# lucidrains/ring-attention-pytorch

Measured on AMD Instinct MI355X. Metric: attn_tflops, higher is better.
Workload: dtype bf16; 1 GPU; model=ring_flash_attn (non-causal, d_head 64), global_batch=1, seq_len=8192, seq_per_gpu=8192, heads=8, kv_heads=8, d_head=64, parallelism=ring1, hipgraph=True

## Files before the change

### ring_attention_amd/csrc/attn_bwd.hip

```cpp

#include <hip/hip_runtime.h>
#include <hip/hip_bf16.h>
#include <cstdint>

#include "attn_common.h"

namespace ring_attn {

template <int D>
struct DqLds {
    static constexpr int KVB = kvblk(D);
    __align__(16) __bf16 k[2][KVB * D];
    __align__(16) __bf16 v[2][KVB * D];
    unsigned char kmask[2][KVB];
};

template <int D, bool SOFTCLAMP, bool PAIRED, bool BIAS = false>
__global__ __launch_bounds__(512, 2)
void attn_bwd_dq_kernel(BwdParams p) {
    constexpr int DBLK = D / 32;
    constexpr int KSTEPS = D / 16;
    constexpr int DQ_KVBLK = kvblk(D);
    constexpr int DQ_NBLK = DQ_KVBLK / 32;

    __shared__ DqLds<D> lds;

    const int tid = threadIdx.x;
    const int lane = tid & 63;
    const int wid = tid >> 6;
    const int l31 = lane & 31;
    const int lhi = lane >> 5;

    const int bh = blockIdx.y;
    const int b = bh / p.h;
    const int h = bh % p.h;
    const int hk = h % p.hk;

    const int n_pit = PAIRED
        ? (p.paired - 1 - (int)blockIdx.x == (int)blockIdx.x ? 1 : 2) : 1;
    for (int pit = 0; pit < n_pit; ++pit) {
    const int qtile = PAIRED
        ? (pit == 0 ? (int)blockIdx.x : p.paired - 1 - (int)blockIdx.x)
        : (p.desc ? p.desc[(long)blockIdx.x * 3] : (int)blockIdx.x);
    if (PAIRED && pit == 1) {
        __syncthreads();
    }

    auto dq_body = [&]() {
    const BwdParams P = p;
    const long i = (long)qtile * ROWS_WG + wid * 32 + l31;
    const bool row_valid = i < P.nq;
    const long ic = row_valid ? i : 0;

    const __bf16* qbase = (const __bf16*)P.q + ((long)b * P.nq + ic) * P.h * D + (long)h * D;
    const __bf16* dobase = (const __bf16*)P.dout + ((long)b * P.nq + ic) * P.h * D + (long)h * D;
    bf16x8 qf[KSTEPS], dof[KSTEPS];
    #pragma unroll
    for (int ks = 0; ks < KSTEPS; ++ks) {
        qf[ks] = *(const bf16x8*)(qbase + ks * 16 + lhi * 8);
        dof[ks] = *(const bf16x8*)(dobase + ks * 16 + lhi * 8);
    }
    const float lse_i = P.lse[((long)b * P.h + h) * P.nq + ic] * LOG2E;
    const float delta_i = P.delta[((long)b * P.h + h) * P.nq + ic];

    f32x16 dq_acc[DBLK];
    #pragma unroll
    for (int db = 0; db < DBLK; ++db) dq_acc[db] = f32x16{};

    const Mask M = mask_of(P);
    const long wg_i_min = (long)qtile * ROWS_WG;
    const long wg_i_max = min((long)(qtile + 1) * ROWS_WG, P.nq) - 1;
    const long wg_q_min = M.qpos(wg_i_min);
    const long wg_q_max = M.qpos(wg_i_max);
    const long qpos_i = M.qpos(i);
    TileRange tr = M.kv_tile_range(wg_i_min, wg_i_max, P.nk, DQ_KVBLK);
    if (P.split > 1) tr = split_share(tr, P.split, (int)blockIdx.z);
    if (!PAIRED && P.desc)
        tr = {P.desc[(long)blockIdx.x * 3 + 1], P.desc[(long)blockIdx.x * 3 + 2]};
    const int t_lo = tr.lo, t_hi = tr.hi;

    constexpr int CH = D * 2 / 16;
    constexpr int KCHUNKS = DQ_KVBLK * CH;
    constexpr int KREGS = (KCHUNKS + 511) / 512;
    const __bf16* kbase = (const __bf16*)P.k + ((long)b * P.nk) * P.hk * D + (long)hk * D;
    const __bf16* vbase = (const __bf16*)P.v + ((long)b * P.nk) * P.hk * D + (long)hk * D;
    const unsigned char* mbase = P.kmask ? (const unsigned char*)P.kmask + (long)b * P.nk : nullptr;

    const long kv_row_stride = (long)P.hk * D;
    const long tile_stride = DQ_KVBLK * kv_row_stride;
    const __bf16* kptr = kbase + (long)t_lo * tile_stride
        + (tid / CH) * kv_row_stride + (tid % CH) * 8;
    const __bf16* vptr = vbase + (long)t_lo * tile_stride
        + (tid / CH) * kv_row_stride + (tid % CH) * 8;
    long j0_next = (long)t_lo * DQ_KVBLK;

    uint4 kst[KREGS], vst[KREGS];
    unsigned char mst = 1;

    auto load_tile = [&]() {
        const long j0 = j0_next;
        const long jmax = min(j0 + DQ_KVBLK, P.nk) - 1;
        const bool full = jmax - j0 == DQ_KVBLK - 1;
        #pragma unroll
        for (int r = 0; r < KREGS; ++r) {
            int c = tid + r * 512;
            if (c < KCHUNKS) {
                long off = (long)(r * (512 / CH)) * kv_row_stride;
                bool okr = full || (j0 + c / CH) <= jmax;
                kst[r] = okr ? *(const uint4*)(kptr + off) : uint4{0, 0, 0, 0};
                vst[r] = okr ? *(const uint4*)(vptr + off) : uint4{0, 0, 0, 0};
            }
        }
        if (mbase && tid < DQ_KVBLK)
            mst = (j0 + tid <= jmax) ? mbase[j0 + tid] : 0;
        kptr += tile_stride; vptr += tile_stride;
        j0_next += DQ_KVBLK;
    };

    auto write_tile = [&](int par) {
        #pragma unroll
        for (int r = 0; r < KREGS; ++r) {
            int c = tid + r * 512;
            if (c < KCHUNKS) {
                int row = c / CH, ch = c % CH;
                *(uint4*)(lds.k[par] + row * D + swz<D / 8>(row, ch) * 8) = kst[r];
                *(uint4*)(lds.v[par] + row * D + swz<D / 8>(row, ch) * 8) = vst[r];
            }
        }
        if (mbase && tid < DQ_KVBLK) lds.kmask[par][tid] = mst;
    };

    const float scale2 = P.scale * LOG2E;
    if (t_lo < t_hi) {
        load_tile();
        write_tile(t_lo & 1);
        if (t_lo + 1 < t_hi) load_tile();
    }

    for (int t = t_lo; t < t_hi; ++t) {
        const int par = t & 1;
        const long j0 = (long)t * DQ_KVBLK;
        const long jmax = min(j0 + DQ_KVBLK, P.nk) - 1;
        const bool full_tile = !BIAS &&
            (jmax - j0 == DQ_KVBLK - 1) &&
            M.uncut(wg_q_min, wg_q_max, j0, jmax) &&
            !P.kmask;

        __syncthreads();

        alignas(16) uint32_t pk[DQ_NBLK * 8];
        __builtin_amdgcn_s_setprio(1);
        #pragma unroll
        for (int kb = 0; kb < DQ_NBLK; ++kb) {
            f32x16 s = f32x16{}, dp = f32x16{};
            int krow = kb * 32 + l31;
            #pragma unroll
            for (int ks = 0; ks < KSTEPS; ++ks) {
                int chunk = ks * 2 + lhi;
                bf16x8 kfr = *(const bf16x8*)(lds.k[par] + krow * D + swz<D / 8>(krow, chunk) * 8);
                bf16x8 vfr = *(const bf16x8*)(lds.v[par] + krow * D + swz<D / 8>(krow, chunk) * 8);
                s = __builtin_amdgcn_mfma_f32_32x32x16_bf16(kfr, qf[ks], s, 0, 0, 0);
                dp = __builtin_amdgcn_mfma_f32_32x32x16_bf16(vfr, dof[ks], dp, 0, 0, 0);
            }
            if (full_tile && row_valid) {
                #pragma unroll
                for (int x2 = 0; x2 < 8; ++x2) {
                    float dse[2];
                    #pragma unroll
                    for (int e = 0; e < 2; ++e) {
                        int r = 2 * x2 + e;
                        float x, dtanh = 1.f;
                        if constexpr (SOFTCLAMP) {
                            float inv_v = __builtin_amdgcn_rcpf(P.softclamp_value);
                            float th = fast_tanhf(s[r] * P.scale * inv_v);
                            x = P.softclamp_value * th * LOG2E;
                            dtanh = 1.f - th * th;
                        } else {
                            x = __builtin_fmaf(s[r], scale2, -lse_i);
                        }
                        float pv = __builtin_amdgcn_exp2f(SOFTCLAMP ? x - lse_i : x);
                        dse[e] = pv * (dp[r] - delta_i);
                        if constexpr (SOFTCLAMP) dse[e] *= dtanh;
                    }
                    pk[kb * 8 + x2] = pack_bf16x2(dse[0], dse[1]);
                }
            } else {
                #pragma unroll
                for (int x2 = 0; x2 < 8; ++x2) {
                    float dse[2];
                    #pragma unroll
                    for (int e = 0; e < 2; ++e) {
                        int r = 2 * x2 + e;
                        long jj = j0 + kb * 32 + (r & 3) + 8 * (r >> 2) + 4 * lhi;
                        float x, dtanh = 1.f;
                        if constexpr (SOFTCLAMP) {
                            float inv_v = __builtin_amdgcn_rcpf(P.softclamp_value);
                            float th = fast_tanhf(s[r] * P.scale * inv_v);
                            x = P.softclamp_value * th * LOG2E;
                            dtanh = 1.f - th * th;
                        } else {
                            x = s[r] * scale2;
                        }
                        bool ok = row_valid && jj <= jmax;
                        if constexpr (BIAS) {
                            if (ok) {
                                const long bi = P.bias_mat
                                    ? (((long)b * P.h + h) * P.nq + ic) * P.nk + jj
                                    : ((long)b * P.h + h) * P.nk + jj;
                                x += P.bias[bi] * LOG2E;
                            }
                        }
                        ok = M.attends(qpos_i, jj, ok);
                        if (P.kmask) ok = ok && lds.kmask[par][jj - j0];
                        float pv = ok ? __builtin_amdgcn_exp2f(
                            SOFTCLAMP ? x - lse_i : x - lse_i) : 0.f;
                        dse[e] = pv * (dp[r] - delta_i);
                        if constexpr (SOFTCLAMP) dse[e] *= dtanh;
                    }
                    pk[kb * 8 + x2] = pack_bf16x2(dse[0], dse[1]);
                }
            }
        }
        __builtin_amdgcn_s_setprio(0);

        if (t + 1 < t_hi) write_tile(par ^ 1);
        if (t + 2 < t_hi) load_tile();

        {
            const int f15 = lane & 15;
            const int g16 = (lane >> 4) & 1;
            const unsigned kb_lds = (unsigned)(uintptr_t)
                (__attribute__((address_space(3))) __bf16*)lds.k[par];
            __builtin_amdgcn_s_setprio(1);
            unsigned long long ktr[DBLK][DQ_NBLK * 2][2];
            #pragma unroll
            for (int db = 0; db < DBLK; ++db) {
                const int dg = db * 32 + g16 * 16 + 4 * (f15 & 3);
                #pragma unroll
                for (int ks = 0; ks < DQ_NBLK * 2; ++ks) {
                    #pragma unroll
                    for (int half = 0; half < 2; ++half) {
                        const int kv = ks * 16 + 4 * lhi + 8 * half + (f15 >> 2);
                        const int c = (dg / 8) ^ (kv & (CH < 8 ? CH - 1 : 7));
                        const unsigned a = kb_lds
                            + (unsigned)(kv * (D * 2) + c * 16 + (dg % 8) * 2);
                        asm volatile("ds_read_b64_tr_b16 %0, %1"
                                     : "=&v"(ktr[db][ks][half]) : "v"(a) : "memory");
                    }
                }
            }
            asm volatile("s_waitcnt lgkmcnt(0)" ::: "memory");
            __builtin_amdgcn_sched_barrier(0);
            #pragma unroll
            for (int db = 0; db < DBLK; ++db)
                #pragma unroll
                for (int ks = 0; ks < DQ_NBLK * 2; ++ks) {
                    bf16x8 ktf;
                    *(unsigned long long*)&ktf = ktr[db][ks][0];
                    *((unsigned long long*)&ktf + 1) = ktr[db][ks][1];
                    dq_acc[db] = __builtin_amdgcn_mfma_f32_32x32x16_bf16(
                        ktf, *(const bf16x8*)(pk + 4 * ks), dq_acc[db], 0, 0, 0);
                }
            __builtin_amdgcn_s_setprio(0);
        }
    }

    if (!row_valid) return;
    #pragma unroll
    for (int db = 0; db < DBLK; ++db) dq_acc[db] *= P.scale;
    if (P.dq_bf) {
        __bf16* dqb = (__bf16*)P.dq_bf + ((long)b * P.nq + i) * P.h * D + (long)h * D;
        #pragma unroll
        for (int db = 0; db < DBLK; ++db)
            #pragma unroll
            for (int g = 0; g < 4; ++g) {
                f32x4 v4 = {dq_acc[db][4 * g], dq_acc[db][4 * g + 1],
                            dq_acc[db][4 * g + 2], dq_acc[db][4 * g + 3]};
                *(bf16x4*)(dqb + db * 32 + 8 * g + 4 * lhi) =
                    __builtin_convertvector(v4, bf16x4);
            }
        return;
    }
    float* dqp = P.dq + ((long)b * P.nq + i) * P.h * D + (long)h * D;
    #pragma unroll
    for (int db = 0; db < DBLK; ++db)
        #pragma unroll
        for (int r = 0; r < 16; ++r) {
            int d = db * 32 + (r & 3) + 8 * (r >> 2) + 4 * lhi;
            if (P.split > 1 || P.desc) atomicAdd(dqp + d, dq_acc[db][r]);
            else if (P.accumulate) dqp[d] += dq_acc[db][r];
            else dqp[d] = dq_acc[db][r];
        }
    };
    dq_body();
    }
}

static constexpr int KVROWS_WAVE = 32;
static_assert(ROWS_WG == 8 * KVROWS_WAVE);

template <int D, int QT>
struct DkvLds {
    __align__(16) __bf16 q[2][QT * D];
    __align__(16) __bf16 qt[2][D * QT];
    __align__(16) __bf16 do_[2][QT * D];
    __align__(16) __bf16 dot[2][D * QT];
    __align__(16) float lse[2][QT];
    __align__(16) float delta[2][QT];
};


template <int D, int QT, bool SOFTCLAMP, bool PAIRED, bool BIAS = false>
__global__ __launch_bounds__(512, 2)
void attn_bwd_dkv_kernel(BwdParams p) {
    static_assert(D % 32 == 0 && QT % 32 == 0);
    constexpr int DBLK = D / 32;
    constexpr int KSTEPS = D / 16;
    constexpr int QBLKS = QT / 32;
    constexpr int TM = (QT / 8 - 1) < 7 ? (QT / 8 - 1) : 7;

    __shared__ DkvLds<D, QT> lds;

    const int tid = threadIdx.x;
    const int lane = tid & 63;
    const int wid = tid >> 6;
    const int l31 = lane & 31;
    const int lhi = lane >> 5;

    const int bhk = blockIdx.y;
    const int b = bhk / p.hk;
    const int hkh = bhk % p.hk;

    const int n_pit = PAIRED
        ? (p.paired - 1 - (int)blockIdx.x == (int)blockIdx.x ? 1 : 2) : 1;
    for (int pit = 0; pit < n_pit; ++pit) {
    const int kvtile = PAIRED
        ? (pit == 0 ? (int)blockIdx.x : p.paired - 1 - (int)blockIdx.x)
        : (p.desc ? p.desc[(long)blockIdx.x * 3] : (int)blockIdx.x);
    if (PAIRED && pit == 1) {
        __syncthreads();
    }

    auto dkv_body = [&]() {
    const BwdParams P = p;
    const long j0_wg = (long)kvtile * ROWS_WG;
    const long jmax = min(j0_wg + ROWS_WG, P.nk) - 1;
    const long j = j0_wg + wid * KVROWS_WAVE + l31;
    const bool col_valid = j <= jmax;
    const long jc = col_valid ? j : j0_wg;

    const __bf16* kb = (const __bf16*)P.k + ((long)b * P.nk + jc) * P.hk * D + (long)hkh * D;
    const __bf16* vb = (const __bf16*)P.v + ((long)b * P.nk + jc) * P.hk * D + (long)hkh * D;
    bf16x8 kf[KSTEPS], vf[KSTEPS];
    #pragma unroll
    for (int ks = 0; ks < KSTEPS; ++ks) {
        kf[ks] = *(const bf16x8*)(kb + ks * 16 + lhi * 8);
        vf[ks] = *(const bf16x8*)(vb + ks * 16 + lhi * 8);
    }
    unsigned char kmask_own = 1;
    if (P.kmask) kmask_own = col_valid ? ((const unsigned char*)P.kmask)[(long)b * P.nk + j] : 0;

    f32x16 dv_acc[DBLK], dk_acc[DBLK];
    #pragma unroll
    for (int db = 0; db < DBLK; ++db) { dv_acc[db] = f32x16{}; dk_acc[db] = f32x16{}; }
    const float scale2 = P.scale * LOG2E;

    const Mask M = mask_of(P);

    for (int g = 0; g < P.group; ++g) {
        if (g > 0) __syncthreads();
        const int h = hkh + g * P.hk;
        const float* lse_row = P.lse + ((long)b * P.h + h) * P.nq;
        const float* delta_row = P.delta + ((long)b * P.h + h) * P.nq;
        const __bf16* qg = (const __bf16*)P.q + ((long)b * P.nq) * P.h * D + (long)h * D;
        const __bf16* dog = (const __bf16*)P.dout + ((long)b * P.nq) * P.h * D + (long)h * D;

        TileRange tr = M.q_tile_range(j0_wg, jmax, P.nq, QT);
        if (P.split > 1) tr = split_share(tr, P.split, (int)blockIdx.z);
        if (!PAIRED && P.desc)
            tr = {P.desc[(long)blockIdx.x * 3 + 1], P.desc[(long)blockIdx.x * 3 + 2]};
        const int t0 = tr.lo, t1 = tr.hi;

        constexpr int CH = D * 2 / 16;
        constexpr int QCHUNKS = QT * CH;
        constexpr int QREGS = (QCHUNKS + 511) / 512;
        constexpr int TPAIRS = (QT / 2) * (D / 8);
        constexpr int TREGS = (TPAIRS + 511) / 512;
        uint4 qst[QREGS], dost[QREGS];
        bf16x8 qtv_a[TREGS], qtv_b[TREGS], dov_a[TREGS], dov_b[TREGS];
        float lse_st = 0.f, delta_st = 0.f;
        long t_next = t0;

        auto load_qtile = [&]() {
            const long i0 = t_next * QT;
            const long imax_ = min(i0 + QT, P.nq) - 1;
            const bool full = imax_ - i0 == QT - 1;
            #pragma unroll
            for (int r = 0; r < QREGS; ++r) {
                int c = tid + r * 512;
                if (c < QCHUNKS) {
                    long gr = i0 + c / CH;
                    int ch = c % CH;
                    const __bf16* src = qg + gr * P.h * D + ch * 8;
                    const __bf16* srd = dog + gr * P.h * D + ch * 8;
                    bool okr = full || gr <= imax_;
                    qst[r] = okr ? *(const uint4*)src : uint4{0, 0, 0, 0};
                    dost[r] = okr ? *(const uint4*)srd : uint4{0, 0, 0, 0};
                }
            }
            #pragma unroll
            for (int r = 0; r < TREGS; ++r) {
                int c = tid + r * 512;
                if (c < TPAIRS) {
                    int jp = c % (QT / 2);
                    int d0 = (c / (QT / 2)) * 8;
                    long ra = i0 + jp * 2;
                    bool oka = full || ra <= imax_;
                    bool okb = full || ra + 1 <= imax_;
                    const __bf16* qa_ = qg + ra * P.h * D + d0;
                    const __bf16* da_ = dog + ra * P.h * D + d0;
                    qtv_a[r] = oka ? *(const bf16x8*)qa_ : bf16x8{};
                    qtv_b[r] = okb ? *(const bf16x8*)(qa_ + P.h * D) : bf16x8{};
                    dov_a[r] = oka ? *(const bf16x8*)da_ : bf16x8{};
                    dov_b[r] = okb ? *(const bf16x8*)(da_ + P.h * D) : bf16x8{};
                }
            }
            if (tid < QT) {
                long gi = i0 + tid;
                bool okl = gi <= imax_;
                lse_st = okl ? lse_row[gi] * LOG2E : 0.f;
                delta_st = okl ? delta_row[gi] : 0.f;
            }
            ++t_next;
        };

        auto write_qtile = [&](int par) {
            #pragma unroll
            for (int r = 0; r < QREGS; ++r) {
                int c = tid + r * 512;
                if (c < QCHUNKS) {
                    int row = c / CH, ch = c % CH;
                    *(uint4*)(lds.q[par] + row * D + swz<D / 8>(row, ch) * 8) = qst[r];
                    *(uint4*)(lds.do_[par] + row * D + swz<D / 8>(row, ch) * 8) = dost[r];
                }
            }
            #pragma unroll
            for (int r = 0; r < TREGS; ++r) {
                int c = tid + r * 512;
                if (c < TPAIRS) {
                    int jp = kperm_pair(c % (QT / 2));
                    int d0 = (c / (QT / 2)) * 8;
                    #pragma unroll
                    for (int e = 0; e < 8; ++e) {
                        int dd = d0 + e;
                        int byte_off = dd * QT * 2 + ((jp * 4) ^ ((dd & TM) << 4));
                        __bf16 pq[2] = {qtv_a[r][e], qtv_b[r][e]};
                        __bf16 pd[2] = {dov_a[r][e], dov_b[r][e]};
                        *(uint32_t*)((char*)lds.qt[par] + byte_off) = *(uint32_t*)pq;
                        *(uint32_t*)((char*)lds.dot[par] + byte_off) = *(uint32_t*)pd;
                    }
                }
            }
            if (tid < QT) {
                lds.lse[par][tid] = lse_st;
                lds.delta[par][tid] = delta_st;
            }
        };

        if (t0 < t1) {
            load_qtile();
            write_qtile(t0 & 1);
            if (t0 + 1 < t1) load_qtile();
        }

        for (int t = t0; t < t1; ++t) {
            const int par = t & 1;
            const long i0 = (long)t * QT;
            const long imax = min(i0 + QT, P.nq) - 1;
            const bool full_tile = !BIAS &&
                (imax - i0 == QT - 1) &&
                M.uncut(M.qpos(i0), M.qpos(imax), j0_wg, jmax) &&
                !P.kmask;

            __syncthreads();

            if (t + 1 < t1) write_qtile(par ^ 1);
            if (t + 2 < t1) load_qtile();

            #pragma unroll
            for (int qb = 0; qb < QBLKS; ++qb) {
                f32x16 s2 = f32x16{}, dp = f32x16{};
                #pragma unroll
                for (int ks = 0; ks < KSTEPS; ++ks) {
                    int qrow = qb * 32 + l31;
                    int chunk = ks * 2 + lhi;
                    bf16x8 qa = *(const bf16x8*)(lds.q[par] + qrow * D + swz<D / 8>(qrow, chunk) * 8);
                    bf16x8 da = *(const bf16x8*)(lds.do_[par] + qrow * D + swz<D / 8>(qrow, chunk) * 8);
                    s2 = __builtin_amdgcn_mfma_f32_32x32x16_bf16(qa, kf[ks], s2, 0, 0, 0);
                    dp = __builtin_amdgcn_mfma_f32_32x32x16_bf16(da, vf[ks], dp, 0, 0, 0);
                }

                alignas(16) uint32_t p_pk[8], ds_pk[8];
                if (full_tile && col_valid) {
                    #pragma unroll
                    for (int x2 = 0; x2 < 8; ++x2) {
                        float pe[2], dse[2];
                        f32x4 lse4, delta4;
                        {
                            int base = qb * 32 + 8 * (x2 >> 1) + 4 * lhi;
                            lse4 = *(const f32x4*)(lds.lse[par] + base);
                            delta4 = *(const f32x4*)(lds.delta[par] + base);
                        }
                        #pragma unroll
                        for (int e = 0; e < 2; ++e) {
                            int r = 2 * x2 + e;
                            float x, dtanh = 1.f;
                            if constexpr (SOFTCLAMP) {
                                float inv_v = __builtin_amdgcn_rcpf(P.softclamp_value);
                                float th = fast_tanhf(s2[r] * P.scale * inv_v);
                                x = P.softclamp_value * th * LOG2E;
                                dtanh = 1.f - th * th;
                            } else {
                                x = __builtin_fmaf(s2[r], scale2, -lse4[r & 3]);
                            }
                            float pv = __builtin_amdgcn_exp2f(SOFTCLAMP ? x - lse4[r & 3] : x);
                            pe[e] = pv;
                            dse[e] = pv * (dp[r] - delta4[r & 3]);
                            if constexpr (SOFTCLAMP) dse[e] *= dtanh;
                        }
                        p_pk[x2] = pack_bf16x2(pe[0], pe[1]);
                        ds_pk[x2] = pack_bf16x2(dse[0], dse[1]);
                    }
                } else {
                    #pragma unroll
                    for (int x2 = 0; x2 < 8; ++x2) {
                        float pe[2], dse[2];
                        f32x4 lse4, delta4;
                        {
                            int base = qb * 32 + 8 * (x2 >> 1) + 4 * lhi;
                            lse4 = *(const f32x4*)(lds.lse[par] + base);
                            delta4 = *(const f32x4*)(lds.delta[par] + base);
                        }
                        #pragma unroll
                        for (int e = 0; e < 2; ++e) {
                            int r = 2 * x2 + e;
                            int qloc = qb * 32 + (r & 3) + 8 * (r >> 2) + 4 * lhi;
                            long i = i0 + qloc;
                            float x, dtanh = 1.f;
                            if constexpr (SOFTCLAMP) {
                                float inv_v = __builtin_amdgcn_rcpf(P.softclamp_value);
                                float th = fast_tanhf(s2[r] * P.scale * inv_v);
                                x = P.softclamp_value * th * LOG2E;
                                dtanh = 1.f - th * th;
                            } else {
                                x = s2[r] * scale2;
                            }
                            bool ok = col_valid && i <= imax;
                            if constexpr (BIAS) {
                                if (ok) {
                                    const long bi = P.bias_mat
                                        ? (((long)b * P.h + h) * P.nq + i) * P.nk + j
                                        : ((long)b * P.h + h) * P.nk + j;
                                    x += P.bias[bi] * LOG2E;
                                }
                            }
                            ok = M.attends(M.qpos(i), j, ok);
                            if (P.kmask) ok = ok && kmask_own;
                            float pv = ok ? __builtin_amdgcn_exp2f(x - lse4[r & 3]) : 0.f;
                            pe[e] = pv;
                            dse[e] = pv * (dp[r] - delta4[r & 3]);
                            if constexpr (SOFTCLAMP) dse[e] *= dtanh;
                        }
                        p_pk[x2] = pack_bf16x2(pe[0], pe[1]);
                        ds_pk[x2] = pack_bf16x2(dse[0], dse[1]);
                    }
                }

                #pragma unroll
                for (int db = 0; db < DBLK; ++db)
                    #pragma unroll
                    for (int half = 0; half < 2; ++half) {
                        int qk = qb * 2 + half;
                        int drow = db * 32 + l31;
                        int ch = qk * 2 + lhi;
                        bf16x8 doa = *(const bf16x8*)(lds.dot[par] + drow * QT +
                                                      ((ch ^ (drow & TM))) * 8);
                        dv_acc[db] = __builtin_amdgcn_mfma_f32_32x32x16_bf16(
                            doa, *(const bf16x8*)(p_pk + 4 * half), dv_acc[db], 0, 0, 0);
                        bf16x8 qta = *(const bf16x8*)(lds.qt[par] + drow * QT +
                                                      ((ch ^ (drow & TM))) * 8);
                        dk_acc[db] = __builtin_amdgcn_mfma_f32_32x32x16_bf16(
                            *(const bf16x8*)(ds_pk + 4 * half), qta, dk_acc[db], 0, 0, 0);
                    }
            }
        }
    }

    #pragma unroll
    for (int db = 0; db < DBLK; ++db) dk_acc[db] *= P.scale;

    if (P.dk_bf) {
        constexpr int ECH = D / 8;
        __bf16* stg_dk = (__bf16*)&lds;
        __bf16* stg_dv = stg_dk + ROWS_WG * D;
        static_assert(sizeof(DkvLds<D, QT>) >= 2 * ROWS_WG * D * sizeof(__bf16));
        const int wrow0 = wid * KVROWS_WAVE;
        const long orow_stride = (long)P.hk * D;
        __bf16* dkb = (__bf16*)P.dk_bf + ((long)b * P.nk) * orow_stride + (long)hkh * D;
        __bf16* dvb = (__bf16*)P.dv_bf + ((long)b * P.nk) * orow_stride + (long)hkh * D;
        __syncthreads();
        #pragma unroll
        for (int db = 0; db < DBLK; ++db)
            #pragma unroll
            for (int r = 0; r < 16; ++r) {
                int row = wrow0 + (r & 3) + 8 * (r >> 2) + 4 * lhi;
                int d = db * 32 + l31;
                stg_dk[row * D + swz<ECH>(row, d / 8) * 8 + (d & 7)] = (__bf16)dk_acc[db][r];
            }
        {
            const int row = wrow0 + l31;
            #pragma unroll
            for (int db = 0; db < DBLK; ++db)
                #pragma unroll
                for (int g = 0; g < 4; ++g) {
                    f32x4 v4 = {dv_acc[db][4 * g], dv_acc[db][4 * g + 1],
                                dv_acc[db][4 * g + 2], dv_acc[db][4 * g + 3]};
                    *(bf16x4*)(stg_dv + row * D + swz<ECH>(row, db * 4 + g) * 8 + 4 * lhi) =
                        __builtin_convertvector(v4, bf16x4);
                }
        }
        __syncthreads();
        #pragma unroll
        for (int c = lane; c < KVROWS_WAVE * ECH; c += 64) {
            int row = wrow0 + c / ECH, ch = c % ECH;
            long kvrow = j0_wg + row;
            if (kvrow <= jmax) {
                int so = row * D + swz<ECH>(row, ch) * 8;
                *(uint4*)(dkb + kvrow * orow_stride + ch * 8) = *(const uint4*)(stg_dk + so);
                *(uint4*)(dvb + kvrow * orow_stride + ch * 8) = *(const uint4*)(stg_dv + so);
            }
        }
    } else {
        float* dkb = P.dk + (((long)b * P.hk + hkh) * P.nk) * D;
        #pragma unroll
        for (int db = 0; db < DBLK; ++db)
            #pragma unroll
            for (int r = 0; r < 16; ++r) {
                long kvrow = j0_wg + wid * KVROWS_WAVE + (r & 3) + 8 * (r >> 2) + 4 * lhi;
                int d = db * 32 + l31;
                if (kvrow <= jmax) {
                    float* dst = dkb + kvrow * D + d;
                    if (P.split > 1 || P.desc) atomicAdd(dst, dk_acc[db][r]);
                    else if (P.accumulate) *dst += dk_acc[db][r];
                    else *dst = dk_acc[db][r];
                }
            }
        float* dvb = P.dv + (((long)b * P.hk + hkh) * D) * P.nk;
        if (col_valid)
        #pragma unroll
        for (int db = 0; db < DBLK; ++db)
            #pragma unroll
            for (int r = 0; r < 16; ++r) {
                int d = db * 32 + (r & 3) + 8 * (r >> 2) + 4 * lhi;
                float* dst = dvb + (long)d * P.nk + j;
                if (P.split > 1 || P.desc) atomicAdd(dst, dv_acc[db][r]);
                else if (P.accumulate) *dst += dv_acc[db][r];
                else *dst = dv_acc[db][r];
            }
    }
    };
    if constexpr (D == 64) noinline_call(dkv_body);
    else dkv_body();
    }
}

void launch_attn_bwd_dq(const BwdParams& p, int head_dim, hipStream_t stream) {
    dim3 block(512);
    int z = p.split > 1 ? p.split : 1;
    long qt_ = ceil_div(p.nq, ROWS_WG);
    if (p.desc) qt_ = p.n_units;
    else if (p.paired) qt_ = (qt_ + 1) / 2;
    dim3 grid_dq(qt_, p.b * p.h, z);
    const bool pr = p.paired > 0;
    if (p.bias) {
        if (head_dim == 64) {
            if (p.softclamp) hipLaunchKernelGGL((attn_bwd_dq_kernel<64, true, false, true>), grid_dq, block, 0, stream, p);
            else hipLaunchKernelGGL((attn_bwd_dq_kernel<64, false, false, true>), grid_dq, block, 0, stream, p);
        } else if (head_dim == 128) {
            if (p.softclamp) hipLaunchKernelGGL((attn_bwd_dq_kernel<128, true, false, true>), grid_dq, block, 0, stream, p);
            else hipLaunchKernelGGL((attn_bwd_dq_kernel<128, false, false, true>), grid_dq, block, 0, stream, p);
        } else {
            if (p.softclamp) hipLaunchKernelGGL((attn_bwd_dq_kernel<32, true, false, true>), grid_dq, block, 0, stream, p);
            else hipLaunchKernelGGL((attn_bwd_dq_kernel<32, false, false, true>), grid_dq, block, 0, stream, p);
        }
        return;
    }
    if (head_dim == 64) {
        if (p.softclamp) if (pr) hipLaunchKernelGGL((attn_bwd_dq_kernel<64, true, true>), grid_dq, block, 0, stream, p);
        else hipLaunchKernelGGL((attn_bwd_dq_kernel<64, true, false>), grid_dq, block, 0, stream, p);
        else if (pr) hipLaunchKernelGGL((attn_bwd_dq_kernel<64, false, true>), grid_dq, block, 0, stream, p);
        else hipLaunchKernelGGL((attn_bwd_dq_kernel<64, false, false>), grid_dq, block, 0, stream, p);
    } else if (head_dim == 128) {
        if (p.softclamp) if (pr) hipLaunchKernelGGL((attn_bwd_dq_kernel<128, true, true>), grid_dq, block, 0, stream, p);
        else hipLaunchKernelGGL((attn_bwd_dq_kernel<128, true, false>), grid_dq, block, 0, stream, p);
        else if (pr) hipLaunchKernelGGL((attn_bwd_dq_kernel<128, false, true>), grid_dq, block, 0, stream, p);
        else hipLaunchKernelGGL((attn_bwd_dq_kernel<128, false, false>), grid_dq, block, 0, stream, p);
    } else if (head_dim == 32) {
        if (p.softclamp) if (pr) hipLaunchKernelGGL((attn_bwd_dq_kernel<32, true, true>), grid_dq, block, 0, stream, p);
        else hipLaunchKernelGGL((attn_bwd_dq_kernel<32, true, false>), grid_dq, block, 0, stream, p);
        else if (pr) hipLaunchKernelGGL((attn_bwd_dq_kernel<32, false, true>), grid_dq, block, 0, stream, p);
        else hipLaunchKernelGGL((attn_bwd_dq_kernel<32, false, false>), grid_dq, block, 0, stream, p);
    } else {
        __builtin_trap();
    }
}

void launch_attn_bwd_dkv(const BwdParams& p, int head_dim, hipStream_t stream) {
    dim3 block(512);
    int z = p.split > 1 ? p.split : 1;
    long kt_ = ceil_div(p.nk, ROWS_WG);
    if (p.desc) kt_ = p.n_units;
    else if (p.paired) kt_ = (kt_ + 1) / 2;
    dim3 grid_dkv(kt_, p.b * p.hk, z);
    const bool pr = p.paired > 0;
    if (p.bias) {
        if (head_dim == 64) {
            if (p.softclamp) hipLaunchKernelGGL((attn_bwd_dkv_kernel<64, DKV_QT, true, false, true>), grid_dkv, block, 0, stream, p);
            else hipLaunchKernelGGL((attn_bwd_dkv_kernel<64, DKV_QT, false, false, true>), grid_dkv, block, 0, stream, p);
        } else if (head_dim == 128) {
            if (p.softclamp) hipLaunchKernelGGL((attn_bwd_dkv_kernel<128, DKV_QT, true, false, true>), grid_dkv, block, 0, stream, p);
            else hipLaunchKernelGGL((attn_bwd_dkv_kernel<128, DKV_QT, false, false, true>), grid_dkv, block, 0, stream, p);
        } else {
            if (p.softclamp) hipLaunchKernelGGL((attn_bwd_dkv_kernel<32, DKV_QT, true, false, true>), grid_dkv, block, 0, stream, p);
            else hipLaunchKernelGGL((attn_bwd_dkv_kernel<32, DKV_QT, false, false, true>), grid_dkv, block, 0, stream, p);
        }
        return;
    }
    if (head_dim == 64) {
        if (p.softclamp) if (pr) hipLaunchKernelGGL((attn_bwd_dkv_kernel<64, DKV_QT, true, true>), grid_dkv, block, 0, stream, p);
        else hipLaunchKernelGGL((attn_bwd_dkv_kernel<64, DKV_QT, true, false>), grid_dkv, block, 0, stream, p);
        else if (pr) hipLaunchKernelGGL((attn_bwd_dkv_kernel<64, DKV_QT, false, true>), grid_dkv, block, 0, stream, p);
        else hipLaunchKernelGGL((attn_bwd_dkv_kernel<64, DKV_QT, false, false>), grid_dkv, block, 0, stream, p);
    } else if (head_dim == 128) {
        if (p.softclamp) if (pr) hipLaunchKernelGGL((attn_bwd_dkv_kernel<128, DKV_QT, true, true>), grid_dkv, block, 0, stream, p);
        else hipLaunchKernelGGL((attn_bwd_dkv_kernel<128, DKV_QT, true, false>), grid_dkv, block, 0, stream, p);
        else if (pr) hipLaunchKernelGGL((attn_bwd_dkv_kernel<128, DKV_QT, false, true>), grid_dkv, block, 0, stream, p);
        else hipLaunchKernelGGL((attn_bwd_dkv_kernel<128, DKV_QT, false, false>), grid_dkv, block, 0, stream, p);
    } else if (head_dim == 32) {
        if (p.softclamp) if (pr) hipLaunchKernelGGL((attn_bwd_dkv_kernel<32, DKV_QT, true, true>), grid_dkv, block, 0, stream, p);
        else hipLaunchKernelGGL((attn_bwd_dkv_kernel<32, DKV_QT, true, false>), grid_dkv, block, 0, stream, p);
        else if (pr) hipLaunchKernelGGL((attn_bwd_dkv_kernel<32, DKV_QT, false, true>), grid_dkv, block, 0, stream, p);
        else hipLaunchKernelGGL((attn_bwd_dkv_kernel<32, DKV_QT, false, false>), grid_dkv, block, 0, stream, p);
    } else {
        __builtin_trap();
    }
}

template <int D>
__global__ __launch_bounds__(256) void attn_delta_kernel(DeltaParams p) {
    constexpr int LPR = D / 8;
    constexpr int RPW = 64 / LPR;
    const int lane = threadIdx.x & 63;
    const int wave = (blockIdx.x * (blockDim.x >> 6)) + (threadIdx.x >> 6);
    const long row = (long)wave * RPW + lane / LPR;
    if (row >= p.rows) return;
    const int c = lane % LPR;

    const __bf16* dop = (const __bf16*)p.dout + row * D + c * 8;
    const __bf16* op = (const __bf16*)p.out + row * D + c * 8;
    bf16x8 a = *(const bf16x8*)dop;
    bf16x8 b = *(const bf16x8*)op;
    float s = 0.f;
    #pragma unroll
    for (int e = 0; e < 8; ++e) s += (float)a[e] * (float)b[e];
    #pragma unroll
    for (int off = LPR / 2; off > 0; off >>= 1) s += __shfl_xor(s, off);
    if (c == 0) {
        const long hh = row % p.h;
        const long bi = row / p.h;
        const long i = bi % p.n, bb = bi / p.n;
        p.delta[(bb * p.h + hh) * p.n + i] = s;
    }
}

void launch_attn_delta(const DeltaParams& p, int head_dim, hipStream_t stream) {
    dim3 block(256);
    if (head_dim == 64) {
        long waves = (p.rows + 7) / 8;
        hipLaunchKernelGGL(attn_delta_kernel<64>, dim3((waves + 3) / 4), block, 0, stream, p);
    } else if (head_dim == 128) {
        long waves = (p.rows + 3) / 4;
        hipLaunchKernelGGL(attn_delta_kernel<128>, dim3((waves + 3) / 4), block, 0, stream, p);
    } else if (head_dim == 32) {
        long waves = (p.rows + 15) / 16;
        hipLaunchKernelGGL(attn_delta_kernel<32>, dim3((waves + 3) / 4), block, 0, stream, p);
    } else {
        __builtin_trap();
    }
}

static constexpr int FIN_ROWS = 64;

__device__ __forceinline__ uint4 fin_pack8(const float* s) {
    f32x4 a = {s[0], s[1], s[2], s[3]}, c = {s[4], s[5], s[6], s[7]};
    union { bf16x4 h[2]; uint4 u; } o;
    o.h[0] = __builtin_convertvector(a, bf16x4);
    o.h[1] = __builtin_convertvector(c, bf16x4);
    return o.u;
}

template <int D>
__global__ __launch_bounds__(256) void attn_bwd_finalize_kernel(BwdFinalizeParams p) {
    constexpr int CH = D / 8;
    constexpr int LDW = FIN_ROWS + 1;
    __shared__ float tile[D * LDW];
    const int tid = threadIdx.x;
    const int which = blockIdx.z;

    if (which == 2) {
        if (!p.dq) return;
        const long nblk = (long)gridDim.x * gridDim.y;
        const long blk = (long)blockIdx.y * gridDim.x + blockIdx.x;
        const long chunks = p.dq_elems / 8;
        for (long c = blk * 256 + tid; c < chunks; c += nblk * 256) {
            float s[8];
            *(f32x4*)s = *(const f32x4*)(p.dq + c * 8);
            *(f32x4*)(s + 4) = *(const f32x4*)(p.dq + c * 8 + 4);
            *(uint4*)((__bf16*)p.dq_bf + c * 8) = fin_pack8(s);
        }
        return;
    }
    if (!p.dk) return;

    const int bb = blockIdx.y / p.hk;
    const int hh = blockIdx.y % p.hk;
    const long n0 = (long)blockIdx.x * FIN_ROWS;
    const int rows = (int)min((long)FIN_ROWS, p.nk - n0);
    const long orow_stride = (long)p.hk * D;

    if (which == 0) {
        const float* src = p.dk + (((long)bb * p.hk + hh) * p.nk + n0) * D;
        __bf16* dst = (__bf16*)p.dk_bf + ((long)bb * p.nk + n0) * orow_stride + (long)hh * D;
        for (int c = tid; c < rows * CH; c += 256) {
            int row = c / CH, ch = c % CH;
            float s[8];
            *(f32x4*)s = *(const f32x4*)(src + (long)row * D + ch * 8);
            *(f32x4*)(s + 4) = *(const f32x4*)(src + (long)row * D + ch * 8 + 4);
            *(uint4*)(dst + row * orow_stride + ch * 8) = fin_pack8(s);
        }
        return;
    }

    const float* src = p.dv + (((long)bb * p.hk + hh) * D) * p.nk + n0;
    for (int c = tid; c < D * FIN_ROWS; c += 256) {
        int d = c / FIN_ROWS, nn = c % FIN_ROWS;
        if (nn < rows) tile[d * LDW + nn] = src[(long)d * p.nk + nn];
    }
    __syncthreads();
    __bf16* dst = (__bf16*)p.dv_bf + ((long)bb * p.nk + n0) * orow_stride + (long)hh * D;
    for (int c = tid; c < rows * CH; c += 256) {
        int row = c / CH, ch = c % CH;
        float s[8];
        #pragma unroll
        for (int e = 0; e < 8; ++e) s[e] = tile[(ch * 8 + e) * LDW + row];
        *(uint4*)(dst + row * orow_stride + ch * 8) = fin_pack8(s);
    }
}

void launch_attn_bwd_finalize(const BwdFinalizeParams& p, int head_dim, hipStream_t stream) {
    dim3 block(256);
    long nx = p.dk ? (p.nk + FIN_ROWS - 1) / FIN_ROWS : 256;
    int ny = p.dk ? p.b * p.hk : 1;
    dim3 grid(nx, ny, p.dq ? 3 : 2);
    if (head_dim == 64) hipLaunchKernelGGL(attn_bwd_finalize_kernel<64>, grid, block, 0, stream, p);
    else if (head_dim == 128) hipLaunchKernelGGL(attn_bwd_finalize_kernel<128>, grid, block, 0, stream, p);
    else if (head_dim == 32) hipLaunchKernelGGL(attn_bwd_finalize_kernel<32>, grid, block, 0, stream, p);
    else __builtin_trap();
}

}
```

### ring_attention_amd/csrc/attn_common.h

```cpp
#pragma once

#include <hip/hip_runtime.h>
#include <cstdint>

#ifdef __HIPCC__
#include <hip/hip_bf16.h>
#endif

#include "attn_mask.h"

namespace ring_attn {

#ifdef __HIPCC__
typedef __bf16 bf16_t;
typedef bf16_t bf16x8 __attribute__((ext_vector_type(8)));
typedef float f32x16 __attribute__((ext_vector_type(16)));
typedef float f32x4 __attribute__((ext_vector_type(4)));
typedef bf16_t bf16x4 __attribute__((ext_vector_type(4)));
typedef unsigned int u32x2 __attribute__((ext_vector_type(2)));
typedef float f32x2 __attribute__((ext_vector_type(2)));
typedef bf16_t bf16x2 __attribute__((ext_vector_type(2)));

__device__ __forceinline__ uint32_t pack_bf16x2(float a, float b) {
    union { bf16x2 h; uint32_t u; } c;
    c.h = __builtin_convertvector(f32x2{a, b}, bf16x2);
    return c.u;
}

__device__ __forceinline__ int kperm_pair(int jp) {
    return (jp & ~6) | ((jp & 4) >> 1) | ((jp & 2) << 1);
}

template <int CH>
__device__ __forceinline__ int swz(int row, int chunk) {
    return chunk ^ (row & (CH < 8 ? CH - 1 : 7));
}

__device__ __forceinline__ float fast_tanhf(float x) {
    float e = __builtin_amdgcn_exp2f(x * 2.885390081777927f);
    return 1.f - 2.f * __builtin_amdgcn_rcpf(e + 1.f);
}

__device__ __forceinline__ float cross_half(float x) {
    union { float f; unsigned u; } c; c.f = x;
    u32x2 r = __builtin_amdgcn_permlane32_swap(c.u, c.u, false, false);
    union { unsigned u; float f; } lo, hi; lo.u = r[0]; hi.u = r[1];
    return (threadIdx.x & 32) ? lo.f : hi.f;
}

template <class F>
__device__ __attribute__((noinline)) void noinline_call(F&& f) { f(); }

static constexpr float LOG2E = 1.4426950408889634f;
static constexpr float LN2 = 0.6931471805599453f;
#endif

static constexpr float MASK_VALUE_F = -3.4028234663852886e38f;

struct FwdParams {
    const void* q;
    const void* k;
    const void* v;
    const void* kmask;
    float* o_acc;
    float* m;
    float* l;
    void* out;
    float* lse;
    int b, h, hk, group;
    long nq, nk;
    float scale;
    float softclamp_value;
    int softclamp;
    int causal;
    long diag;
    long q_stride;
    long win;
    int has_win;
    int is_first;
    int is_last;
    int kv_split;
    int ablate;
    int paired;
    unsigned long long* ticks;
    const float* bias;
    int bias_mat;
};

struct FwdMergeParams {
    const float* o_part;
    const float* m_part;
    const float* l_part;
    float* o_acc;
    float* m;
    float* l;
    void* out;
    float* lse;
    int splits;
    int b, h;
    long nq;
    int is_first;
    int is_last;
};

void launch_attn_fwd_merge(const FwdMergeParams& p, int head_dim, hipStream_t stream);

void launch_attn_fwd(const FwdParams& p, int head_dim, hipStream_t stream);

bool launch_attn_fwd_v2(const FwdParams& p, int head_dim, hipStream_t stream);

struct BwdParams {
    const void* q;
    const void* k;
    const void* v;
    const void* dout;
    const void* kmask;
    const float* lse;
    const float* delta;
    float* dq;
    float* dk;
    float* dv;
    void* dq_bf;
    void* dk_bf;
    void* dv_bf;
    int b, h, hk, group;
    long nq, nk;
    float scale;
    float softclamp_value;
    int softclamp;
    int causal;
    long diag;
    long q_stride;
    long win;
    int has_win;
    int accumulate;
    int split;
    int paired;
    const float* bias;
    int bias_mat;
    const int* desc;
    long n_units;
};

void launch_attn_bwd_dq(const BwdParams& p, int head_dim, hipStream_t stream);
void launch_attn_bwd_dkv(const BwdParams& p, int head_dim, hipStream_t stream);

struct BwdFinalizeParams {
    const float* dk;
    const float* dv;
    const float* dq;
    void* dk_bf;
    void* dv_bf;
    void* dq_bf;
    int b, hk;
    long nk;
    long dq_elems;
};

void launch_attn_bwd_finalize(const BwdFinalizeParams& p, int head_dim, hipStream_t stream);

struct DeltaParams {
    const void* dout;
    const void* out;
    float* delta;
    long rows;
    long n;
    int h;
};

void launch_attn_delta(const DeltaParams& p, int head_dim, hipStream_t stream);

struct DecodeParams {
    const void* q;
    const void* k;
    const void* v;
    float* out;
    float* lse;
    int b, h;
    int hk;
    int nq;
    long n;
    float scale;
    long chunks;
    const void* kscale;
    const void* vscale;
};

void launch_decode_partial(const DecodeParams& p, int head_dim, hipStream_t stream);
void launch_decode_partial_fp8(const DecodeParams& p, int head_dim, hipStream_t stream);

struct DecodeMergeParams {
    const float* outs;
    const float* lses;
    float* out;
    float* lse;
    long rows;
    int s;
};

void launch_decode_merge(const DecodeMergeParams& p, int head_dim, hipStream_t stream);

struct PagedDecodeParams {
    const void* q;
    const void* k_pages;
    const void* v_pages;
    const void* kscale;
    const void* vscale;
    const int* block_table;
    const int* seq_lens;
    float* out;
    float* lse;
    int b, h;
    int hk;
    int nq;
    int page_shift;
    int max_pages;
    int num_pages;
    int causal;
    int chunk_major;
    float scale;
    long chunks;
    long max_seq_len;
};

void launch_decode_partial_paged(const PagedDecodeParams& p, int head_dim, bool fp8,
                                 hipStream_t stream);

struct PagedAppendParams {
    const void* k_new;
    const void* v_new;
    void* k_pages;
    void* v_pages;
    void* kscale;
    void* vscale;
    const int* block_table;
    const int* seq_lens;
    const int* append_lens;
    int b, hk, t;
    int page_shift, max_pages, num_pages;
};

void launch_paged_kv_append(const PagedAppendParams& p, int head_dim, bool fp8,
                            hipStream_t stream);

struct Fp8FwdParams {
    const void* q;
    const void* k;
    const void* vt;
    const void* qs;
    const void* ks;
    const void* vs;
    void* out;
    float* lse;
    int b, h, hk;
    long nq, nk;
    long nk_true;
    int nvs;
    float scale;
    int causal;
    int paired;
};

void launch_attn_fwd_fp8(const Fp8FwdParams& p, int head_dim, hipStream_t stream);

struct RotaryParams {
    const void* x;
    const float* cos_t;
    const float* sin_t;
    void* out;
    long rows;
    int n, h, d;
    float sin_sign;
};

void launch_rotary(const RotaryParams& p, int head_dim, hipStream_t stream);

}
```

Baseline: 395.2 TFLOP/s.

## Prefetch LDS operands and pass kernarg pointer into noinline dkv body

After: 445.4 TFLOP/s, median of 6. +12.7%, better.

```diff
diff --git a/ring_attention_amd/csrc/attn_bwd.hip b/ring_attention_amd/csrc/attn_bwd.hip
--- a/ring_attention_amd/csrc/attn_bwd.hip
+++ b/ring_attention_amd/csrc/attn_bwd.hip
@@ -321,28 +321,45 @@
 
     __shared__ DkvLds<D, QT> lds;
 
-    const int tid = threadIdx.x;
-    const int lane = tid & 63;
-    const int wid = tid >> 6;
-    const int l31 = lane & 31;
-    const int lhi = lane >> 5;
-
-    const int bhk = blockIdx.y;
-    const int b = bhk / p.hk;
-    const int hkh = bhk % p.hk;
+    constexpr bool FRAME = (D == 64);
+    constexpr bool PREFETCH = (D == 64);
 
     const int n_pit = PAIRED
         ? (p.paired - 1 - (int)blockIdx.x == (int)blockIdx.x ? 1 : 2) : 1;
     for (int pit = 0; pit < n_pit; ++pit) {
-    const int kvtile = PAIRED
+    const int kvtile_wg = PAIRED
         ? (pit == 0 ? (int)blockIdx.x : p.paired - 1 - (int)blockIdx.x)
         : (p.desc ? p.desc[(long)blockIdx.x * 3] : (int)blockIdx.x);
     if (PAIRED && pit == 1) {
         __syncthreads();
     }
 
-    auto dkv_body = [&]() {
-    const BwdParams P = p;
+    auto dkv_body = [&](int kvtile_arg, unsigned long long kernarg) {
+    const BwdParams P = [&] {
+        if constexpr (FRAME) {
+            BwdParams kp = kernarg_params<BwdParams>(kernarg);
+            kp.q = as_global(kp.q);         kp.k = as_global(kp.k);
+            kp.v = as_global(kp.v);         kp.dout = as_global(kp.dout);
+            kp.kmask = as_global(kp.kmask); kp.lse = as_global(kp.lse);
+            kp.delta = as_global(kp.delta); kp.dk = as_global(kp.dk);
+            kp.dv = as_global(kp.dv);       kp.dk_bf = as_global(kp.dk_bf);
+            kp.dv_bf = as_global(kp.dv_bf); kp.bias = as_global(kp.bias);
+            kp.desc = as_global(kp.desc);
+            return kp;
+        } else {
+            return p;
+        }
+    }();
+    const int kvtile = uniform<FRAME>(kvtile_arg);
+    const int tid = threadIdx.x;
+    const int lane = tid & 63;
+    const int wid = uniform<FRAME>(tid >> 6);
+    const int l31 = lane & 31;
+    const int lhi = lane >> 5;
+    const int bhk = blockIdx.y;
+    const int b = bhk / P.hk;
+    const int hkh = bhk % P.hk;
+
     const long j0_wg = (long)kvtile * ROWS_WG;
     const long jmax = min(j0_wg + ROWS_WG, P.nk) - 1;
     const long j = j0_wg + wid * KVROWS_WAVE + l31;
@@ -367,6 +384,8 @@
 
     const Mask M = mask_of(P);
 
+    if constexpr (FRAME) __builtin_amdgcn_s_waitcnt(0x0F70);
+
     for (int g = 0; g < P.group; ++g) {
         if (g > 0) __syncthreads();
         const int h = hkh + g * P.hk;
@@ -378,7 +397,8 @@
         TileRange tr = M.q_tile_range(j0_wg, jmax, P.nq, QT);
         if (P.split > 1) tr = split_share(tr, P.split, (int)blockIdx.z);
         if (!PAIRED && P.desc)
-            tr = {P.desc[(long)blockIdx.x * 3 + 1], P.desc[(long)blockIdx.x * 3 + 2]};
+            tr = {uniform<FRAME>(P.desc[(long)blockIdx.x * 3 + 1]),
+                  uniform<FRAME>(P.desc[(long)blockIdx.x * 3 + 2])};
         const int t0 = tr.lo, t1 = tr.hi;
 
         constexpr int CH = D * 2 / 16;
@@ -391,21 +411,30 @@
         float lse_st = 0.f, delta_st = 0.f;
         long t_next = t0;
 
-        auto load_qtile = [&]() {
+        const unsigned qrow_bytes = (unsigned)(P.h * D) * 2u;
+        auto ld16 = [](const __bf16* base, unsigned boff) {
+            return *(const uint4*)((const char*)base + boff);
+        };
+        auto ld8h = [](const __bf16* base, unsigned boff) {
+            return *(const bf16x8*)((const char*)base + boff);
+        };
+        auto tile_rows = [&](long tile) {
+            return (int)(min((tile + 1) * QT, P.nq) - tile * QT);
+        };
+        auto load_qtile = [&](int tid) {
             const long i0 = t_next * QT;
-            const long imax_ = min(i0 + QT, P.nq) - 1;
-            const bool full = imax_ - i0 == QT - 1;
+            const int last = tile_rows(t_next) - 1;
+            const __bf16* qtile = qg + i0 * P.h * D;
+            const __bf16* dotile = dog + i0 * P.h * D;
             #pragma unroll
             for (int r = 0; r < QREGS; ++r) {
                 int c = tid + r * 512;
                 if (c < QCHUNKS) {
-                    long gr = i0 + c / CH;
+                    int lr = min(c / CH, last);
                     int ch = c % CH;
-                    const __bf16* src = qg + gr * P.h * D + ch * 8;
-                    const __bf16* srd = dog + gr * P.h * D + ch * 8;
-                    bool okr = full || gr <= imax_;
-                    qst[r] = okr ? *(const uint4*)src : uint4{0, 0, 0, 0};
-                    dost[r] = okr ? *(const uint4*)srd : uint4{0, 0, 0, 0};
+                    unsigned off = (unsigned)lr * qrow_bytes + ch * 16;
+                    qst[r] = ld16(qtile, off);
+                    dost[r] = ld16(dotile, off);
                 }
             }
             #pragma unroll
@@ -414,27 +443,38 @@
                 if (c < TPAIRS) {
                     int jp = c % (QT / 2);
                     int d0 = (c / (QT / 2)) * 8;
-                    long ra = i0 + jp * 2;
-                    bool oka = full || ra <= imax_;
-                    bool okb = full || ra + 1 <= imax_;
-                    const __bf16* qa_ = qg + ra * P.h * D + d0;
-                    const __bf16* da_ = dog + ra * P.h * D + d0;
-                    qtv_a[r] = oka ? *(const bf16x8*)qa_ : bf16x8{};
-                    qtv_b[r] = okb ? *(const bf16x8*)(qa_ + P.h * D) : bf16x8{};
-                    dov_a[r] = oka ? *(const bf16x8*)da_ : bf16x8{};
-                    dov_b[r] = okb ? *(const bf16x8*)(da_ + P.h * D) : bf16x8{};
+                    unsigned offa = (unsigned)min(jp * 2, last) * qrow_bytes + d0 * 2;
+                    unsigned offb = (unsigned)min(jp * 2 + 1, last) * qrow_bytes + d0 * 2;
+                    qtv_a[r] = ld8h(qtile, offa);
+                    qtv_b[r] = ld8h(qtile, offb);
+                    dov_a[r] = ld8h(dotile, offa);
+                    dov_b[r] = ld8h(dotile, offb);
                 }
             }
             if (tid < QT) {
-                long gi = i0 + tid;
-                bool okl = gi <= imax_;
-                lse_st = okl ? lse_row[gi] * LOG2E : 0.f;
-                delta_st = okl ? delta_row[gi] : 0.f;
+                long gi = i0 + min(tid, last);
+                lse_st = lse_row[gi];
+                delta_st = delta_row[gi];
             }
             ++t_next;
         };
 
-        auto write_qtile = [&](int par) {
+        auto write_qtile = [&](int par, int tid, long tile) {
+            const int rows = tile_rows(tile);
+            if (rows < QT) {
+                #pragma unroll
+                for (int r = 0; r < QREGS; ++r)
+                    if ((tid + r * 512) / CH >= rows) {
+                        qst[r] = uint4{0, 0, 0, 0};
+                        dost[r] = uint4{0, 0, 0, 0};
+                    }
+                #pragma unroll
+                for (int r = 0; r < TREGS; ++r) {
+                    int la = ((tid + r * 512) % (QT / 2)) * 2;
+                    if (la >= rows) { qtv_a[r] = bf16x8{}; dov_a[r] = bf16x8{}; }
+                    if (la + 1 >= rows) { qtv_b[r] = bf16x8{}; dov_b[r] = bf16x8{}; }
+                }
+            }
             #pragma unroll
             for (int r = 0; r < QREGS; ++r) {
                 int c = tid + r * 512;
@@ -450,27 +490,29 @@
                 if (c < TPAIRS) {
                     int jp = kperm_pair(c % (QT / 2));
                     int d0 = (c / (QT / 2)) * 8;
+                    static_assert((TM << 4) < QT * 2 && (D * QT * 2) % (QT * 2) == 0);
+                    const unsigned base = par * (D * QT * 2) + d0 * QT * 2 + jp * 4;
                     #pragma unroll
                     for (int e = 0; e < 8; ++e) {
-                        int dd = d0 + e;
-                        int byte_off = dd * QT * 2 + ((jp * 4) ^ ((dd & TM) << 4));
+                        unsigned byte_off = (base ^ ((e & TM) << 4)) + e * QT * 2;
                         __bf16 pq[2] = {qtv_a[r][e], qtv_b[r][e]};
                         __bf16 pd[2] = {dov_a[r][e], dov_b[r][e]};
-                        *(uint32_t*)((char*)lds.qt[par] + byte_off) = *(uint32_t*)pq;
-                        *(uint32_t*)((char*)lds.dot[par] + byte_off) = *(uint32_t*)pd;
+                        *(uint32_t*)((char*)lds.qt[0] + byte_off) = *(uint32_t*)pq;
+                        *(uint32_t*)((char*)lds.dot[0] + byte_off) = *(uint32_t*)pd;
                     }
                 }
             }
             if (tid < QT) {
-                lds.lse[par][tid] = lse_st;
-                lds.delta[par][tid] = delta_st;
+                const bool okl = tid < rows;
+                lds.lse[par][tid] = okl ? lse_st * LOG2E : 0.f;
+                lds.delta[par][tid] = okl ? delta_st : 0.f;
             }
         };
 
         if (t0 < t1) {
-            load_qtile();
-            write_qtile(t0 & 1);
-            if (t0 + 1 < t1) load_qtile();
+            load_qtile(tid);
+            write_qtile(t0 & 1, tid, t0);
+            if (t0 + 1 < t1) load_qtile(tid);
         }
 
         for (int t = t0; t < t1; ++t) {
@@ -482,22 +524,64 @@
                 M.uncut(M.qpos(i0), M.qpos(imax), j0_wg, jmax) &&
                 !P.kmask;
 
-            __syncthreads();
-
-            if (t + 1 < t1) write_qtile(par ^ 1);
-            if (t + 2 < t1) load_qtile();
-
-            #pragma unroll
-            for (int qb = 0; qb < QBLKS; ++qb) {
-                f32x16 s2 = f32x16{}, dp = f32x16{};
+            bf16x8 qa[KSTEPS], da[KSTEPS], doa[2 * DBLK], qta[2 * DBLK];
+            auto read_sdp = [&](int qb) {
                 #pragma unroll
                 for (int ks = 0; ks < KSTEPS; ++ks) {
                     int qrow = qb * 32 + l31;
                     int chunk = ks * 2 + lhi;
-                    bf16x8 qa = *(const bf16x8*)(lds.q[par] + qrow * D + swz<D / 8>(qrow, chunk) * 8);
-                    bf16x8 da = *(const bf16x8*)(lds.do_[par] + qrow * D + swz<D / 8>(qrow, chunk) * 8);
-                    s2 = __builtin_amdgcn_mfma_f32_32x32x16_bf16(qa, kf[ks], s2, 0, 0, 0);
-                    dp = __builtin_amdgcn_mfma_f32_32x32x16_bf16(da, vf[ks], dp, 0, 0, 0);
+                    qa[ks] = *(const bf16x8*)(lds.q[par] + qrow * D + swz<D / 8>(qrow, chunk) * 8);
+                    da[ks] = *(const bf16x8*)(lds.do_[par] + qrow * D + swz<D / 8>(qrow, chunk) * 8);
+                }
+            };
+            auto read_dvdk = [&](int qb) {
+                #pragma unroll
+                for (int db = 0; db < DBLK; ++db)
+                    #pragma unroll
+                    for (int half = 0; half < 2; ++half) {
+                        int qk = qb * 2 + half;
+                        int drow = db * 32 + l31;
+                        int ch = qk * 2 + lhi;
+                        doa[db * 2 + half] = *(const bf16x8*)(lds.dot[par] + drow * QT +
+                                                              ((ch ^ (drow & TM))) * 8);
+                        qta[db * 2 + half] = *(const bf16x8*)(lds.qt[par] + drow * QT +
+                                                              ((ch ^ (drow & TM))) * 8);
+                    }
+            };
+
+            const int rows_m1 = (int)(imax - i0);
+            int lhi4 = 4 * lhi;
+            asm volatile("" : "+v"(lhi4));
+            long qp_lane = M.qpos(i0 + lhi4);
+            asm volatile("" : "+v"(qp_lane));
+
+            __syncthreads();
+
+            if constexpr (PREFETCH) {
+                read_sdp(0);
+                __builtin_amdgcn_sched_barrier(0);
+            }
+
+            int tid_l = tid;
+            if constexpr (FRAME) asm volatile("" : "+v"(tid_l));
+            if (t + 1 < t1) write_qtile(par ^ 1, tid_l, t + 1);
+            if (t + 2 < t1) load_qtile(tid_l);
+
+            #pragma unroll
+            for (int qb = 0; qb < QBLKS; ++qb) {
+                f32x16 s2 = f32x16{}, dp = f32x16{};
+                if constexpr (!PREFETCH) read_sdp(qb);
+                #pragma unroll
+                for (int ks = 0; ks < KSTEPS; ++ks) {
+                    s2 = __builtin_amdgcn_mfma_f32_32x32x16_bf16(qa[ks], kf[ks], s2, 0, 0, 0);
+                    dp = __builtin_amdgcn_mfma_f32_32x32x16_bf16(da[ks], vf[ks], dp, 0, 0, 0);
+                }
+                f32x4 lse_g0 = f32x4{}, delta_g0 = f32x4{};
+                if constexpr (PREFETCH) {
+                    lse_g0 = *(const f32x4*)(lds.lse[par] + qb * 32 + 4 * lhi);
+                    delta_g0 = *(const f32x4*)(lds.delta[par] + qb * 32 + 4 * lhi);
+                    read_dvdk(qb);
+                    __builtin_amdgcn_sched_barrier(0);
                 }
 
                 alignas(16) uint32_t p_pk[8], ds_pk[8];
@@ -506,7 +590,10 @@
                     for (int x2 = 0; x2 < 8; ++x2) {
                         float pe[2], dse[2];
                         f32x4 lse4, delta4;
-                        {
+                        if (PREFETCH && (x2 >> 1) == 0) {
+                            lse4 = lse_g0;
+                            delta4 = delta_g0;
+                        } else {
                             int base = qb * 32 + 8 * (x2 >> 1) + 4 * lhi;
                             lse4 = *(const f32x4*)(lds.lse[par] + base);
                             delta4 = *(const f32x4*)(lds.delta[par] + base);
@@ -536,7 +623,10 @@
                     for (int x2 = 0; x2 < 8; ++x2) {
                         float pe[2], dse[2];
                         f32x4 lse4, delta4;
-                        {
+                        if (PREFETCH && (x2 >> 1) == 0) {
+                            lse4 = lse_g0;
+                            delta4 = delta_g0;
+                        } else {
                             int base = qb * 32 + 8 * (x2 >> 1) + 4 * lhi;
                             lse4 = *(const f32x4*)(lds.lse[par] + base);
                             delta4 = *(const f32x4*)(lds.delta[par] + base);
@@ -544,8 +634,8 @@
                         #pragma unroll
                         for (int e = 0; e < 2; ++e) {
                             int r = 2 * x2 + e;
-                            int qloc = qb * 32 + (r & 3) + 8 * (r >> 2) + 4 * lhi;
-                            long i = i0 + qloc;
+                            const int cr = qb * 32 + (r & 3) + 8 * (r >> 2);
+                            const int qloc = cr + lhi4;
                             float x, dtanh = 1.f;
                             if constexpr (SOFTCLAMP) {
                                 float inv_v = __builtin_amdgcn_rcpf(P.softclamp_value);
@@ -555,16 +645,17 @@
                             } else {
                                 x = s2[r] * scale2;
                             }
-                            bool ok = col_valid && i <= imax;
+                            bool ok = col_valid && qloc <= rows_m1;
                             if constexpr (BIAS) {
                                 if (ok) {
+                                    const long i = i0 + qloc;
                                     const long bi = P.bias_mat
                                         ? (((long)b * P.h + h) * P.nq + i) * P.nk + j
                                         : ((long)b * P.h + h) * P.nk + j;
                                     x += P.bias[bi] * LOG2E;
                                 }
                             }
-                            ok = M.attends(M.qpos(i), j, ok);
+                            ok = M.attends(qp_lane + (long)cr * M.q_stride, j, ok);
                             if (P.kmask) ok = ok && kmask_own;
                             float pv = ok ? __builtin_amdgcn_exp2f(x - lse4[r & 3]) : 0.f;
                             pe[e] = pv;
@@ -576,21 +667,22 @@
                     }
                 }
 
+                if constexpr (PREFETCH) {
+                    if (qb + 1 < QBLKS) {
+                        read_sdp(qb + 1);
+                        __builtin_amdgcn_sched_barrier(0);
+                    }
+                } else {
+                    read_dvdk(qb);
+                }
                 #pragma unroll
                 for (int db = 0; db < DBLK; ++db)
                     #pragma unroll
                     for (int half = 0; half < 2; ++half) {
-                        int qk = qb * 2 + half;
-                        int drow = db * 32 + l31;
-                        int ch = qk * 2 + lhi;
-                        bf16x8 doa = *(const bf16x8*)(lds.dot[par] + drow * QT +
-                                                      ((ch ^ (drow & TM))) * 8);
                         dv_acc[db] = __builtin_amdgcn_mfma_f32_32x32x16_bf16(
-                            doa, *(const bf16x8*)(p_pk + 4 * half), dv_acc[db], 0, 0, 0);
-                        bf16x8 qta = *(const bf16x8*)(lds.qt[par] + drow * QT +
-                                                      ((ch ^ (drow & TM))) * 8);
+                            doa[db * 2 + half], *(const bf16x8*)(p_pk + 4 * half), dv_acc[db], 0, 0, 0);
                         dk_acc[db] = __builtin_amdgcn_mfma_f32_32x32x16_bf16(
-                            *(const bf16x8*)(ds_pk + 4 * half), qta, dk_acc[db], 0, 0, 0);
+                            *(const bf16x8*)(ds_pk + 4 * half), qta[db * 2 + half], dk_acc[db], 0, 0, 0);
                     }
             }
         }
@@ -669,8 +761,8 @@
             }
     }
     };
-    if constexpr (D == 64) noinline_call(dkv_body);
-    else dkv_body();
+    if constexpr (FRAME) noinline_call(dkv_body, kvtile_wg, kernarg_address());
+    else dkv_body(kvtile_wg, 0ull);
     }
 }
 
diff --git a/ring_attention_amd/csrc/attn_common.h b/ring_attention_amd/csrc/attn_common.h
--- a/ring_attention_amd/csrc/attn_common.h
+++ b/ring_attention_amd/csrc/attn_common.h
@@ -50,6 +50,38 @@
 
 template <class F>
 __device__ __attribute__((noinline)) void noinline_call(F&& f) { f(); }
+
+template <class F>
+__device__ __attribute__((noinline, not_tail_called))
+void noinline_call(F&& f, int x, unsigned long long kernarg) { f(x, kernarg); }
+
+template <bool ON>
+__device__ __forceinline__ int uniform(int x) {
+    if constexpr (ON) return __builtin_amdgcn_readfirstlane(x);
+    else return x;
+}
+
+__device__ __forceinline__ unsigned long long kernarg_address() {
+    return (unsigned long long)__builtin_amdgcn_kernarg_segment_ptr();
+}
+
+template <class T>
+__device__ __forceinline__ T kernarg_params(unsigned long long kernarg) {
+    static_assert(sizeof(T) % 4 == 0);
+    typedef const __attribute__((address_space(4))) unsigned int* const_words;
+    const unsigned lo = __builtin_amdgcn_readfirstlane((unsigned)kernarg);
+    const unsigned hi = __builtin_amdgcn_readfirstlane((unsigned)(kernarg >> 32));
+    const_words src = (const_words)(((unsigned long long)hi << 32) | lo);
+    union { T t; unsigned w[sizeof(T) / 4]; } u;
+    #pragma unroll
+    for (unsigned i = 0; i < sizeof(T) / 4; ++i) u.w[i] = src[i];
+    return u.t;
+}
+
+template <class T>
+__device__ __forceinline__ T* as_global(T* p) {
+    return (T*)(__attribute__((address_space(1))) T*)(unsigned long long)p;
+}
 
 static constexpr float LOG2E = 1.4426950408889634f;
 static constexpr float LN2 = 0.6931471805599453f;
```
